# olegroshka/vae-channel-dynamics

Hardware: AMD Instinct MI355X
Metric: images/sec SDXL-VAE train step @256x256 (tracking on) (higher is better)
Workload: dtype f32

## Files before the change

include/vaehip.h:

```cpp
#ifndef VAEHIP_H
#define VAEHIP_H
#include <stdint.h>
#ifdef __cplusplus
extern "C" {
#endif

#define VAE_OK 0
#define VAE_EINVAL (-1)
#define VAE_ELAUNCH (-2)

const char* vae_last_error(void);
int vae_abi_version(void);
int vae_sizeof_args(int32_t which);
int vae_set_option(const char* name, int32_t value);
int vae_get_option(const char* name);

#define VAE_XF_NONE 0
#define VAE_XF_AFFINE 1
#define VAE_XF_AFFINE_SILU 2

#define VAE_PREC_F32 0
#define VAE_PREC_BF16 1

#define VAE_MODE_FWD 0
// ... 59 lines not shown
  const float* scale; const float* shift;
  vae_conv_geom g;
  int32_t M, N;
  int32_t ldy;
  int32_t npix;
  int32_t nsplit;
  int32_t batch; int64_t sYb, sXb, sOb;
  int32_t xf;
  float alpha;
  int32_t prec;
  const void* X16;
  const void* dY16;
  int32_t tapmask;
  int32_t y_step, y_oy, y_ox;
  int32_t x_bf16, y_bf16;
} vae_wgrad_args;
int vae_wgrad(const vae_wgrad_args* a, void* stream);
int vae_wgrad_wino_plan(const vae_wgrad_args* a, int32_t* nsplit);
int vae_wgrad_wino(const vae_wgrad_args* a, void* stream);
int vae_wgrad_wino_reduce(const float* slab, int32_t nsplit, int32_t npos, int32_t Cin, int32_t Cout, float* scratch, float* dW,
                          const float* bias_partial, float* db, void* stream);
int vae_wgrad_wino_positions(const vae_wgrad_args* a);
int vae_wgrad_io16_ok(const vae_wgrad_args* a);
int vae_wgrad_phase_ok(const vae_wgrad_args* a);
int vae_upconv_fold_wgrad(const float* dWeff, const float* dbeff, int32_t Co, int32_t Ci, float* dW, float* db, void* stream);
int vae_wgrad_plan(const vae_wgrad_args* a, int32_t* nsplit, int32_t* xf_fusable);
int vae_igemm_kernel_name(const vae_igemm_args* a, char* buf, int32_t n);
int vae_wgrad_kernel_name(const vae_wgrad_args* a, char* buf, int32_t n);
int vae_reduce_splits(const float* partial, int32_t nsplit, int64_t n, float* out, void* stream);
int vae_reduce_splits2(const float* partial, int32_t nsplit, int64_t n, float* out, const float* partial2, int32_t n2, float* out2,
// ... 78 lines not shown
```

vae-channel-dynamics_amd/csrc/common_host.h:

```cpp
#pragma once
#include <stddef.h>
#include <stdint.h>
#include <hip/hip_runtime_api.h>
#include "../../include/vaehip.h"

void vae_set_error(const char* fmt, ...);

#define VAE_CHECK(cond, ...)                 \
  do {                                       \
    if (!(cond)) {                           \
      vae_set_error(__VA_ARGS__);            \
      return VAE_EINVAL;                     \
    }                                        \
  } while (0)

#define VAE_LAUNCH_CHECK(name)                                                 \
  do {                                                                         \
    hipError_t e_ = hipGetLastError();                                         \
    if (e_ != hipSuccess) {                                                    \
      vae_set_error("%s: launch failed: %s", name, hipGetErrorString(e_));     \
      return VAE_ELAUNCH;                                                      \
    }                                                                          \
  } while (0)

static inline bool aligned16(const void* p) { return (((uintptr_t)p) & 15u) == 0; }

constexpr int SS_HALF = 512;
constexpr size_t BUF_MAX = 0xFFFFFFF0u;

struct vae_options {
  int flat_conv;
  int no_wino;
  int no_wino4;
  int no_thin_mfma;
  int no_wide;
  int no_wgrad_dma;
  int wide_reserved_cus;
};
const vae_options& vae_opt();

#define VAE_RESERVE_LDS(kern, bytes, what)                                                                                  \
  do {                                                                                                                      \
    static unsigned long long done_ = 0;                                                                                    \
    int dev_ = 0;                                                                                                           \
    (void)hipGetDevice(&dev_);                                                                                              \
    if (!((done_ >> (dev_ & 63)) & 1ull)) {                                                                                 \
      if (hipFuncSetAttribute(reinterpret_cast<const void*>(kern), hipFuncAttributeMaxDynamicSharedMemorySize, (int)(bytes)) != hipSuccess) { \
        vae_set_error("%s: cannot reserve %d bytes of LDS", what, (int)(bytes));                                            \
        return VAE_ELAUNCH;                                                                                                 \
      }                                                                                                                     \
// ... 4 lines not shown
```

vae-channel-dynamics_amd/csrc/dispatch.cpp:

```cpp
#include <stdio.h>
#include <algorithm>
#include "launchers.h"

namespace {

constexpr int BK = 32;
const char* const TF[2] = {"false", "true"};

int check_geom(const char* who, const vae_conv_geom& g) {
  VAE_CHECK(g.B > 0 && g.Hs > 0 && g.Ws > 0 && g.Cs > 0 && g.Ho > 0 && g.Wo > 0, "%s: non-positive geometry", who);
  VAE_CHECK(g.taps == 1 || g.taps == 9, "%s: taps must be 1 or 9 (got %d)", who, g.taps);
  VAE_CHECK(g.stride == 1 || g.stride == 2, "%s: stride must be 1 or 2", who);
  VAE_CHECK(g.mode >= 0 && g.mode <= 4, "%s: bad mode", who);
  VAE_CHECK(g.mode != VAE_MODE_UP2X_DGRAD || (g.taps == 9 && g.stride == 1 && g.Hs == 2 * g.Ho && g.Ws == 2 * g.Wo),
            "%s: UP2X_DGRAD needs 3x3 stride 1, source twice the row grid", who);
  VAE_CHECK(g.mode != VAE_MODE_DGRAD_S2 ||
                (g.taps == 9 && g.stride == 2 && g.pad_t == 0 && g.pad_l == 0 && g.Ho % 2 == 0 && g.Wo % 2 == 0 &&
                 ((int64_t)g.B * g.Ho * g.Wo / 4) % 128 == 0),
            "%s: DGRAD_S2 needs 3x3 stride 2 pad 0, even row grid and B*Ho*Wo/4 %% 128 == 0", who);
  VAE_CHECK(g.mode != VAE_MODE_UP2X || (g.taps == 9 && g.stride == 1), "%s: up2x needs 3x3 stride 1", who);
  return 0;
}

bool xf_rows_ok(const vae_conv_geom& g, int M, int K) {
// ... 477 lines not shown
  const char* what = "wgrad";
  switch (s.k) {
    case WgradKernel::DmaBf16: rc = launch_wgrad3_dma_bf16(a, st); what = "wgrad3_dma_bf16"; break;
    case WgradKernel::TileBf16: rc = launch_wgrad3_tile_bf16(a, st); what = "wgrad3_tile_bf16"; break;
    case WgradKernel::Tile: rc = launch_wgrad3_tile(a, st); what = "wgrad3_tile"; break;
    case WgradKernel::ThinBf16: rc = launch_wgrad_thin(a, st); what = "wgrad_thin_bf16"; break;
    case WgradKernel::SmallK: rc = launch_wgrad_smallk(a, st); what = "wgrad_smallk"; break;
    case WgradKernel::Bf16: rc = launch_wgrad_bf16(a, st); what = "wgrad_bf16"; break;
    default: rc = launch_wgrad_f32(a, s.vec, st); break;
  }
  if (rc) return rc;
  VAE_LAUNCH_CHECK(what);
  return VAE_OK;
}

extern "C" int vae_wgrad_wino_plan(const vae_wgrad_args* ap, int32_t* nsplit) {
  VAE_CHECK(ap && nsplit, "wgrad_wino_plan: null argument");
  *nsplit = 0;
  if (vae_opt().flat_conv || vae_opt().no_wino) return VAE_OK;
  const bool up = wgrad3_upwino_eligible(*ap);
  if (!up && !wgrad3_wino_eligible(*ap)) return VAE_OK;
  const int64_t units = up ? wgrad3_upwino_units(ap->g) : wgrad3_wino_units(ap->g);
  const int64_t wgs = (int64_t)(ap->M / 128) * (ap->N / 32);
  *nsplit = (int32_t)std::max<int64_t>(1, std::min<int64_t>(256 / std::max<int64_t>(wgs, 1), units / 8));
  return VAE_OK;
}
extern "C" int vae_wgrad_wino_positions(const vae_wgrad_args* ap) { return (ap && wgrad3_upwino_eligible(*ap)) ? 9 : 16; }
extern "C" int vae_wgrad_wino(const vae_wgrad_args* ap, void* stream) {
  VAE_CHECK(ap != nullptr, "wgrad_wino: null args");
  const vae_wgrad_args& a = *ap;
  if (int e = check_geom("wgrad_wino", a.g)) return e;
  VAE_CHECK(a.dY && a.X && a.partial, "wgrad_wino: null operand");
  VAE_CHECK(a.nsplit > 0 && a.nsplit <= 65535, "wgrad_wino: bad nsplit");
  VAE_CHECK((int64_t)a.g.B * a.g.Ho * a.g.Wo == a.npix && a.N <= a.g.Cs && a.ldy >= a.M, "wgrad_wino: inconsistent sizes");
  const bool up = wgrad3_upwino_eligible(a);
  if (!up) {
    VAE_CHECK(wgrad3_wino_eligible(a), "wgrad_wino: the layer is not served by the Winograd kernel (vae_wgrad_wino_plan)");
    VAE_CHECK(a.xf == VAE_XF_NONE || (a.scale && a.shift), "wgrad_wino: xf needs scale/shift");
  }
  if (int rc = (up ? launch_wgrad3_upwino : launch_wgrad3_wino)(a, (hipStream_t)stream)) return rc;
  VAE_LAUNCH_CHECK(up ? "wgrad3_upwino" : "wgrad3_wino");
  return VAE_OK;
}
```

vae-channel-dynamics_amd/csrc/error.cpp:

```cpp
#include <stdarg.h>
#include <stdio.h>
#include <stdlib.h>
#include <string.h>
#include "common_host.h"

static thread_local char g_err[512] = "";

void vae_set_error(const char* fmt, ...) {
  va_list ap;
  va_start(ap, fmt);
  vsnprintf(g_err, sizeof(g_err), fmt, ap);
  va_end(ap);
}

static vae_options init_options() {
  vae_options o;
  o.flat_conv = getenv("VAEHIP_FLAT_CONV") ? 1 : 0;
  o.no_wino = getenv("VAEHIP_NO_WINO") ? 1 : 0;
  o.no_wide = getenv("VAEHIP_NO_WIDE") ? 1 : 0;
  o.no_wino4 = getenv("VAEHIP_NO_WINO4") ? 1 : 0;
  o.no_thin_mfma = getenv("VAEHIP_NO_THIN_MFMA") ? 1 : 0;
  o.no_wgrad_dma = getenv("VAEHIP_NO_WGRAD_DMA") ? 1 : 0;
  const char* r = getenv("VAEHIP_WIDE_RESERVED_CUS");
  o.wide_reserved_cus = r ? atoi(r) : 0;
  if (o.wide_reserved_cus < 0 || o.wide_reserved_cus > 128) o.wide_reserved_cus = 0;
  return o;
}
static vae_options g_opt = init_options();
const vae_options& vae_opt() { return g_opt; }

static int* option_slot(const char* name) {
  if (!name) return nullptr;
  if (!strcmp(name, "flat_conv")) return &g_opt.flat_conv;
  if (!strcmp(name, "no_wino")) return &g_opt.no_wino;
  if (!strcmp(name, "no_wide")) return &g_opt.no_wide;
  if (!strcmp(name, "no_wino4")) return &g_opt.no_wino4;
  if (!strcmp(name, "no_thin_mfma")) return &g_opt.no_thin_mfma;
  if (!strcmp(name, "no_wgrad_dma")) return &g_opt.no_wgrad_dma;
  if (!strcmp(name, "wide_reserved_cus")) return &g_opt.wide_reserved_cus;
  return nullptr;
}

extern "C" const char* vae_last_error(void) { return g_err; }
extern "C" int vae_abi_version(void) { return 12; }
extern "C" int vae_sizeof_args(int32_t which) {
  return which == 0 ? (int)sizeof(vae_conv_geom) : which == 1 ? (int)sizeof(vae_igemm_args) : which == 2 ? (int)sizeof(vae_wgrad_args) : -1;
}
extern "C" int vae_set_option(const char* name, int32_t value) {
  int* s = option_slot(name);
  if (!s) {
    vae_set_error("set_option: unknown option '%s' (flat_conv, no_wino, no_wino4, no_wide, no_thin_mfma, no_wgrad_dma, wide_reserved_cus)", name ? name : "(null)");
    return VAE_EINVAL;
  }
  if (s == &g_opt.wide_reserved_cus) {
    if (value < 0 || value > 128) {
      vae_set_error("set_option: wide_reserved_cus must be in 0..128, got %d", (int)value);
      return VAE_EINVAL;
    }
    *s = value;
    return VAE_OK;
  }
  *s = value ? 1 : 0;
  return VAE_OK;
}
extern "C" int vae_get_option(const char* name) {
  int* s = option_slot(name);
// ... 3 lines not shown
```

vae-channel-dynamics_amd/csrc/igemm.hip:

```cpp
#include "common.h"
#include <algorithm>
#include <stdlib.h>

#include "launchers.h"

namespace {

constexpr int BK = 32;
__device__ __forceinline__ int b_lo_of(int m0, int hw) { return m0 / hw; }


template <int BM, int BN, int WM, int WN, bool BKM, bool VEC, int XF>
__global__ __launch_bounds__(64 * WM * WN) void igemm_rows_kernel(vae_igemm_args p) {
  constexpr int NT = 64 * WM * WN;
  constexpr int NL = NT;
  constexpr int RP = NT / 8;
  constexpr int LDA = BK + 4;
  constexpr int LDB = BKM ? (BN + 4) : (BK + 4);
  constexpr int SA = BM * LDA;
  constexpr int SB = BKM ? BK * LDB : BN * LDB;
  constexpr int STAGE = SA + SB;
  constexpr int SS = (XF != VAE_XF_NONE) ? 2 * SS_HALF : 0;
  constexpr int TM = BM / WM, TN = BN / WN, MI = TM / 32, NI = TN / 32;
  constexpr int AR = BM / RP;
// ... 580 lines not shown
  VAE_CHECK(partial && out && nsplit > 0 && n > 0, "reduce_splits: bad args");
  if (int rc = reduce_splits_impl(partial, nsplit, n, out, nullptr, 0, nullptr, (hipStream_t)stream)) return rc;
  VAE_LAUNCH_CHECK("reduce_splits");
  return VAE_OK;
}
extern "C" int vae_reduce_splits2(const float* partial, int32_t nsplit, int64_t n, float* out, const float* partial2, int32_t n2, float* out2,
                                  void* stream) {
  VAE_CHECK(partial && out && partial2 && out2 && nsplit > 0 && n > 0 && n2 > 0, "reduce_splits2: bad args");
  if (int rc = reduce_splits_impl(partial, nsplit, n, out, partial2, n2, out2, (hipStream_t)stream)) return rc;
  VAE_LAUNCH_CHECK("reduce_splits2");
  return VAE_OK;
}
extern "C" int vae_wgrad_wino_reduce(const float* slab, int32_t nsplit, int32_t npos, int32_t Cin, int32_t Cout, float* scratch, float* dW,
                                     const float* bias_partial, float* db, void* stream) {
  VAE_CHECK(slab && dW && nsplit > 0 && Cin > 0 && Cout > 0 && Cin % 32 == 0 && Cout % 32 == 0, "wgrad_wino_reduce: bad args");
  VAE_CHECK(npos == 16 || npos == 9, "wgrad_wino_reduce: npos must be 16 (plain 3x3 layer) or 9 (upsampler convolution)");
  VAE_CHECK((bias_partial == nullptr) == (db == nullptr), "wgrad_wino_reduce: bias_partial and db go together");
  VAE_CHECK(nsplit == 1 || scratch != nullptr, "wgrad_wino_reduce: nsplit > 1 needs the [16*Cin*Cout] scratch buffer");
  hipStream_t st = (hipStream_t)stream;
  if (nsplit > 1) {
    if (int rc = reduce_splits_impl(slab, nsplit, (int64_t)npos * Cin * Cout, scratch, bias_partial, bias_partial ? Cout : 0, db, st)) return rc;
    VAE_LAUNCH_CHECK("reduce_splits");
    if (int rc = (npos == 9 ? launch_upwino_wgrad_reduce : launch_wino_wgrad_reduce)(scratch, 1, Cin, Cout, dW, nullptr, nullptr, st)) return rc;
  } else {
    if (int rc = (npos == 9 ? launch_upwino_wgrad_reduce : launch_wino_wgrad_reduce)(slab, 1, Cin, Cout, dW, bias_partial, db, st)) return rc;
  }
  VAE_LAUNCH_CHECK("wino_wgrad_reduce");
  return VAE_OK;
}
```

vae-channel-dynamics_amd/csrc/launchers.h:

```cpp
#pragma once
#include "common_host.h"

int launch_rows_f32(const vae_igemm_args& a, bool bkm, bool vec, hipStream_t st);
int launch_wgrad_f32(const vae_wgrad_args& a, bool vec, hipStream_t st);
int launch_rows_bf16(const vae_igemm_args& a, bool bkm, hipStream_t st);
int launch_wgrad_bf16(const vae_wgrad_args& a, hipStream_t st);

bool conv3_tile_eligible(const vae_igemm_args& a, bool vec, bool bkm);
int conv3_tile_gstat_chunks(const vae_igemm_args& a);
int launch_conv3_tile(const vae_igemm_args& a, bool bkm, hipStream_t st);
bool conv3_tile_bf16_packed(const vae_igemm_args& a);
int conv3_tile_bf16_gstat_chunks(const vae_igemm_args& a);
int launch_conv3_tile_bf16(const vae_igemm_args& a, bool bkm, hipStream_t st);
bool conv3_wide_bf16_eligible(const vae_igemm_args& a);
int conv3_wide_bf16_gstat_chunks(const vae_igemm_args& a);
int launch_conv3_wide_bf16(const vae_igemm_args& a, hipStream_t st);
bool conv3_wino_eligible(const vae_igemm_args& a);
int conv3_wino_nb();
int conv3_wino_gstat_chunks(const vae_igemm_args& a);
int conv3_wino_gnb_chunks(const vae_igemm_args& a);
int launch_wino_weights(const vae_igemm_args& a, float* U, hipStream_t st);
int launch_conv3_wino(const vae_igemm_args& a, const float* U, hipStream_t st);
bool conv3_wino4_eligible(const vae_igemm_args& a);
int conv3_wino4_gstat_chunks(const vae_igemm_args& a);
// ... 19 lines not shown
bool wgrad_thin_bf16_eligible(const vae_wgrad_args& a, int kind);
int launch_wgrad_thin(const vae_wgrad_args& a, hipStream_t st);

bool wgrad3_tile_eligible(const vae_wgrad_args& a, bool vec);
int64_t wgrad3_tile_units(const vae_conv_geom& g);
int launch_wgrad3_tile(const vae_wgrad_args& a, hipStream_t st);
bool wgrad3_dma_bf16_operands(const vae_wgrad_args& a);
bool wgrad3_tile_bf16_eligible(const vae_wgrad_args& a, bool vec, bool dma);
int64_t wgrad3_tile_bf16_units(const vae_conv_geom& g);
int wgrad3_tile_bf16_columns(const vae_wgrad_args& a);
int launch_wgrad3_tile_bf16(const vae_wgrad_args& a, hipStream_t st);
int launch_wgrad3_dma_bf16(const vae_wgrad_args& a, hipStream_t st);
bool wgrad3_wino_eligible(const vae_wgrad_args& a);
int64_t wgrad3_wino_units(const vae_conv_geom& g);
int launch_wgrad3_wino(const vae_wgrad_args& a, hipStream_t st);
int launch_wino_wgrad_reduce(const float* slab, int nsplit, int N, int M, float* dW, const float* bpart, float* db, hipStream_t st);
bool wgrad3_upwino_eligible(const vae_wgrad_args& a);
int64_t wgrad3_upwino_units(const vae_conv_geom& g);
int launch_wgrad3_upwino(const vae_wgrad_args& a, hipStream_t st);
int launch_upwino_wgrad_reduce(const float* slab, int nsplit, int N, int M, float* dW, const float* bpart, float* db, hipStream_t st);
```

vae-channel-dynamics_amd/src/vaehip/engine.py:

```python
from __future__ import annotations

import contextlib
import weakref
from typing import Callable, Dict, List, Optional

import torch
import torch.nn as nn

from . import ops
from .ops import XF_AFFINE, XF_AFFINE_SILU, XF_NONE, Stats

_TRACK_C = {4, 8, 16, 32, 64, 128, 256, 512, 1024}
MOMENT_METRICS = ("mean_abs_activation_per_channel", "mean_activation", "std_activation")
DEVICE_METRICS = MOMENT_METRICS + ("full_activation_map",)


class _TrackHandle:
    def __init__(self, store: dict, key, point: str, sink):
        self._s, self._k, self._p, self._f = store, key, point, sink

    def remove(self):
        lst = self._s.get(self._k, {}).get(self._p, [])
        if self._f in lst:
            lst.remove(self._f)
# ... 239 lines not shown

    def _take16(self, recording: bool) -> Optional[torch.Tensor]:
        a16, self._last16 = self._last16, None
        return a16 if recording else None

    def _conv_bwd(self, m, x, dy, xf, st, need_dx=True, x16=None, dx_to_gn=False, dx_dtype=None, norm=None):
        kind = getattr(m, "kind", "c1")
        gnb = None
        if norm is not None and need_dx and st is not None and xf in (XF_AFFINE, XF_AFFINE_SILU):
            gnb = ops.GnCtx(x, st, norm.weight, norm.bias, xf == XF_AFFINE_SILU, norm.num_groups)
        if (need_dx and dy.dtype == torch.float32 and getattr(dy, "_b16", None) is None
                and ops.grad_image_ok(kind, x.shape[:3] + (m.weight.shape[1],), m.weight.shape[0], m.weight.shape[1])):
            dy._b16 = ops.pack_bf16(dy, torch.empty(dy.shape, device=dy.device, dtype=torch.bfloat16))
        if x16 is not None and x16.dtype == torch.float32:
            x, xf, st, x16 = x16, XF_NONE, None, None
        ops.conv_wgrad(dy, x, kind, self._g(m.weight), self._g(m.bias), xf=xf, stats=st, x16=x16)
        if need_dx:
            return ops.conv_dgrad(dy, m.weight, kind, (x.shape[1], x.shape[2]), out_bf16=dx_to_gn, out_dtype=dx_dtype, gnb=gnb)
        return None

    def _gn_bwd(self, norm, x, g, st, silu, add, conv_only=None, feeds_conv3=False):
        want32, want16 = True, False
        if ops.act16():
            want32, want16 = False, True
        elif conv_only is not None and ops.grad_image_ok(getattr(conv_only, "kind", "c1"), x.shape[:3] + (conv_only.weight.shape[1],),
                                                      conv_only.weight.shape[0], conv_only.weight.shape[1]):
            want32, want16 = False, True
        elif feeds_conv3 and ops.grad_image_ok("c3", x.shape, x.shape[3], x.shape[3]):
            want16 = True
        return ops.gn_bwd(x, g, st, norm.weight, norm.bias, silu, add, self._g(norm.weight), self._g(norm.bias),
                          norm.num_groups, want32=want32, want16=want16)
# ... 346 lines not shown
```

vae-channel-dynamics_amd/src/vaehip/lib.py:

```python
from __future__ import annotations

import ctypes as C
import os

_HERE = os.path.dirname(os.path.abspath(__file__))
LIB_PATH = os.environ.get("VAEHIP_LIB") or os.path.normpath(os.path.join(_HERE, "..", "..", "csrc", "libvaehip.so"))


class VaeHipError(RuntimeError):
    pass


class ConvGeom(C.Structure):
    _fields_ = [("B", C.c_int32), ("Hs", C.c_int32), ("Ws", C.c_int32), ("Cs", C.c_int32),
                ("Ho", C.c_int32), ("Wo", C.c_int32), ("taps", C.c_int32), ("stride", C.c_int32),
                ("pad_t", C.c_int32), ("pad_l", C.c_int32), ("mode", C.c_int32)]


_fp = C.c_void_p


class IgemmArgs(C.Structure):
    _fields_ = [("A", _fp), ("W", _fp), ("C", _fp), ("bias", _fp), ("res", _fp), ("scale", _fp), ("shift", _fp),
                ("track", _fp), ("g", ConvGeom), ("M", C.c_int32), ("N", C.c_int32), ("K", C.c_int32),
# ... 2 lines not shown
                ("xf", C.c_int32), ("alpha", C.c_float), ("prec", C.c_int32), ("Wh", _fp), ("A16", _fp),
                ("tapmask", C.c_int32), ("a_step", C.c_int32), ("a_oy", C.c_int32), ("a_ox", C.c_int32),
                ("c_step", C.c_int32), ("c_oy", C.c_int32), ("c_ox", C.c_int32),
                ("gstat", _fp), ("gstat_groups", C.c_int32), ("Wu", _fp), ("out_bf16", C.c_int32),
                ("a_bf16", C.c_int32), ("res_bf16", C.c_int32),
                ("gnb_x", _fp), ("gnb_mean", _fp), ("gnb_rstd", _fp), ("gnb_gamma", _fp), ("gnb_beta", _fp), ("gnb_ws", _fp),
                ("gnb_groups", C.c_int32), ("gnb_silu", C.c_int32), ("gnb_x_bf16", C.c_int32)]


class WgradArgs(C.Structure):
    _fields_ = [("dY", _fp), ("X", _fp), ("out", _fp), ("partial", _fp), ("bias_partial", _fp), ("scale", _fp), ("shift", _fp),
                ("g", ConvGeom), ("M", C.c_int32), ("N", C.c_int32), ("ldy", C.c_int32), ("npix", C.c_int32),
                ("nsplit", C.c_int32), ("batch", C.c_int32), ("sYb", C.c_int64), ("sXb", C.c_int64),
                ("sOb", C.c_int64), ("xf", C.c_int32), ("alpha", C.c_float), ("prec", C.c_int32), ("X16", _fp), ("dY16", _fp),
                ("tapmask", C.c_int32), ("y_step", C.c_int32), ("y_oy", C.c_int32), ("y_ox", C.c_int32),
                ("x_bf16", C.c_int32), ("y_bf16", C.c_int32)]


i32, i64, f32, vp = C.c_int32, C.c_int64, C.c_float, C.c_void_p
EXPECTED_ABI = 12

SIGNATURES = {
    "vae_set_option": [C.c_char_p, i32],
    "vae_get_option": [C.c_char_p],
    "vae_igemm_rows": [C.POINTER(IgemmArgs), vp],
    "vae_conv_gstat_chunks": [C.POINTER(IgemmArgs)],
    "vae_conv_gnb_chunks": [C.POINTER(IgemmArgs)],
    "vae_conv_phase_ok": [C.POINTER(IgemmArgs)],
    "vae_conv_io16_ok": [C.POINTER(IgemmArgs)],
    "vae_wgrad_io16_ok": [C.POINTER(WgradArgs)],
    "vae_add_bf16": [vp, vp, i64, vp, vp],
    "vae_unpack_bf16": [vp, i64, vp, vp],
    "vae_wino_ok": [C.POINTER(IgemmArgs)],
    "vae_wino_weight_floats": [C.POINTER(IgemmArgs)],
    "vae_wino_weights": [C.POINTER(IgemmArgs), vp, vp],
# ... 101 lines not shown
```

vae-channel-dynamics_amd/src/vaehip/ops.py:

```python
from __future__ import annotations

import ctypes as C
import os
from typing import NamedTuple, Optional, Tuple

import torch

from .lib import ConvGeom, IgemmArgs, WgradArgs, lib

XF_NONE, XF_AFFINE, XF_AFFINE_SILU = 0, 1, 2
PREC_F32, PREC_BF16 = 0, 1
PRECISION = PREC_F32


FUSED_GN_STATS = True

WEIGHTS16: Optional[Tuple[int, int, int]] = None


def pack_bf16(src: torch.Tensor, dst: torch.Tensor) -> torch.Tensor:
    assert src.is_contiguous() and dst.is_contiguous() and dst.numel() == src.numel() and dst.element_size() == 2
    lib.call("vae_pack_bf16", _p(src), src.numel(), _p(dst), _stream())
    return dst

# ... 631 lines not shown
            else:
                a.partial = _p(partial)
            a.bias_partial = _p(bpart)
            _launch_wgrad(a)
            if ns > 1 and bpart is not None:
                lib.call("vae_reduce_splits2", _p(partial), ns, n, _p(dwe[ph]), _p(bpart), Co, _p(dbe[ph]), _stream())
            elif ns > 1:
                lib.call("vae_reduce_splits", _p(partial), ns, n, _p(dwe[ph]), _stream())
            elif bpart is not None:
                lib.call("vae_reduce_splits", _p(bpart), ns, Co, _p(dbe[ph]), _stream())
    lib.call("vae_upconv_fold_wgrad", _p(dwe), _p(dbe), Co, Ci, _p(gv), _p(bgrad_out), _stream())
    del keep
    return True


def _wgrad_wino(a: WgradArgs, gv: torch.Tensor, bgrad_out: Optional[torch.Tensor], dev) -> bool:
    if not WINOGRAD or PRECISION != PREC_F32:
        return False
    ns = C.c_int32(0)
    lib.call("vae_wgrad_wino_plan", C.byref(a), C.byref(ns))
    ns = ns.value
    if ns <= 0:
        return False
    npos = int(lib.query("vae_wgrad_wino_positions", C.byref(a)))
    slab = torch.empty((ns, npos * a.N * a.M), device=dev, dtype=torch.float32)
    bpart = torch.empty((ns, a.M), device=dev, dtype=torch.float32) if bgrad_out is not None else None
    a.nsplit, a.partial, a.bias_partial = ns, _p(slab), _p(bpart)
    fl = 2.0 * a.M * a.N * a.npix * 9
    if npos == 9:
        _timed("wgrad3_upwino_kernel", fl, fl * 0.25, "vae_wgrad_wino", C.byref(a), _stream())
    else:
        _timed(f"wgrad3_wino_kernel<{a.xf}>", fl, fl * WINO_EXECUTED, "vae_wgrad_wino", C.byref(a), _stream())
    scratch = torch.empty((npos * a.N * a.M,), device=dev, dtype=torch.float32) if ns > 1 else None
    _timed("wgrad_wino_reduce (split sum + output transform)", 0.0, 0.0, "vae_wgrad_wino_reduce", _p(slab), ns, npos, a.N, a.M,
           _p(scratch), _p(gv), _p(bpart), _p(bgrad_out), _stream())
    return True


def conv_wgrad(dy: torch.Tensor, x: torch.Tensor, kind: str, wgrad_out: torch.Tensor,
               bgrad_out: Optional[torch.Tensor], *, xf: int = XF_NONE, stats: Optional[Stats] = None,
               x16: Optional[torch.Tensor] = None):
    dy16 = _grad16(dy)
    dy32 = dy if dy.dtype == torch.float32 else None
    _chk_act(dy, "conv_wgrad.dy")
    _chk_act(x, "conv_wgrad.x")
    if x16 is not None:
        assert x16.shape == x.shape and x16.dtype == torch.bfloat16 and x16.is_contiguous()
        xf = XF_NONE
    gv = ohwi(wgrad_out)
    Co, kh, kw, Ci = gv.shape
    taps = kh * kw
    B, H, W, Cs = x.shape
    g = _fwd_geom(kind, B, H, W, Cs)
    assert dy.shape == (B, g.Ho, g.Wo, Co), (dy.shape, (B, g.Ho, g.Wo, Co))
    if (kind == "c3up" and PRECISION == PREC_F32 and WINOGRAD and xf == XF_NONE and x16 is None and dy32 is not None
            and x.dtype == torch.float32):
# ... 13 lines not shown
    a.dY, a.X = _p(dy32 if dy32 is not None else dy16), _p(x)
    a.dY16 = _p(dy16) if use16 else None
    a.g = g
    a.M, a.N, a.ldy, a.npix, a.nsplit = Co, Ci, Co, npix, 1
    a.batch, a.sYb, a.sXb, a.sOb = 1, 0, 0, 0
    a.xf, a.alpha, a.prec = xf, 1.0, PRECISION
    if x16 is not None:
        a.X16 = _p(x16)
    elif xb and xf == XF_NONE:
        a.X16 = _p(x)
    elif xb:
        a.x_bf16 = 1
    if xf != XF_NONE:
        assert stats is not None
        a.scale, a.shift = _p(stats.scale), _p(stats.shift)
    if _wgrad_wino(a, gv, bgrad_out, x.device):
        return
    ns, fus = C.c_int32(0), C.c_int32(0)
    lib.call("vae_wgrad_plan", C.byref(a), C.byref(ns), C.byref(fus))
    if xf != XF_NONE and not fus.value:
        x = gn_apply(x, stats, xf)
        a.X, a.xf, a.scale, a.shift, a.x_bf16 = _p(x), XF_NONE, None, None, 0
        lib.call("vae_wgrad_plan", C.byref(a), C.byref(ns), C.byref(fus))
    if (a.X16 or a.dY16 or a.x_bf16) and not lib.query("vae_wgrad_io16_ok", C.byref(a)):
        x32 = to_f32(x16) if x16 is not None else to_f32(x)
        return conv_wgrad(dy32 if dy32 is not None else to_f32(dy16), x32, kind, wgrad_out, bgrad_out, xf=xf, stats=stats)
    ns = ns.value
    a.nsplit = ns
    partial = None
    if ns == 1:
        a.out = _p(gv)
# ... 318 lines not shown
```

Measured before the change: 103.6.

## Add Winograd F(4x4,3x3) weight-gradient kernel for large f32 3x3 convolutions

Adds a new Winograd F(4,3) weight-gradient path with 36 transform positions for plain stride-1 3x3 f32 layers whose output is at least 64x64. It is used when the engine requests wino4 and no fused GroupNorm transform is involved. A warp-specialised kernel transforms input and output-gradient tiles in LDS and accumulates them with MFMA into split slabs. A second kernel sums the splits and applies the inverse transform to produce dW and db. The goal is fewer multiplies than the existing F(2,3) Winograd path or the direct wgrad on high-resolution layers, at the cost of larger slab and scratch buffers, more transform work, and possible f32 precision loss from the F(4,3) transform constants.

After: 107.2 (median of 6 runs). +3.4%, better.

```diff
diff --git a/include/vaehip.h b/include/vaehip.h
--- a/include/vaehip.h
+++ b/include/vaehip.h
@@ -97,6 +97,7 @@
   int32_t tapmask;
   int32_t y_step, y_oy, y_ox;
   int32_t x_bf16, y_bf16;
+  int32_t wino4;
 } vae_wgrad_args;
 int vae_wgrad(const vae_wgrad_args* a, void* stream);
 int vae_wgrad_wino_plan(const vae_wgrad_args* a, int32_t* nsplit);
diff --git a/vae-channel-dynamics_amd/csrc/common_host.h b/vae-channel-dynamics_amd/csrc/common_host.h
--- a/vae-channel-dynamics_amd/csrc/common_host.h
+++ b/vae-channel-dynamics_amd/csrc/common_host.h
@@ -34,6 +34,7 @@
   int no_wino4;
   int no_thin_mfma;
   int no_wide;
+  int no_wgrad_wino4;
   int no_wgrad_dma;
   int wide_reserved_cus;
 };
diff --git a/vae-channel-dynamics_amd/csrc/dispatch.cpp b/vae-channel-dynamics_amd/csrc/dispatch.cpp
--- a/vae-channel-dynamics_amd/csrc/dispatch.cpp
+++ b/vae-channel-dynamics_amd/csrc/dispatch.cpp
@@ -515,10 +515,18 @@
   return VAE_OK;
 }
 
+static bool wgrad_use_wino4(const vae_wgrad_args& a) {
+  return a.wino4 != 0 && (int64_t)a.g.Ho * a.g.Wo >= 64 * 64 && !vae_opt().flat_conv && !vae_opt().no_wino && !vae_opt().no_wgrad_wino4 && !wgrad3_upwino_eligible(a) &&
+         wgrad3_wino4_eligible(a);
+}
 extern "C" int vae_wgrad_wino_plan(const vae_wgrad_args* ap, int32_t* nsplit) {
   VAE_CHECK(ap && nsplit, "wgrad_wino_plan: null argument");
   *nsplit = 0;
   if (vae_opt().flat_conv || vae_opt().no_wino) return VAE_OK;
+  if (wgrad_use_wino4(*ap)) {
+    *nsplit = wgrad3_wino4_nsplit(*ap);
+    return VAE_OK;
+  }
   const bool up = wgrad3_upwino_eligible(*ap);
   if (!up && !wgrad3_wino_eligible(*ap)) return VAE_OK;
   const int64_t units = up ? wgrad3_upwino_units(ap->g) : wgrad3_wino_units(ap->g);
@@ -526,7 +534,9 @@
   *nsplit = (int32_t)std::max<int64_t>(1, std::min<int64_t>(256 / std::max<int64_t>(wgs, 1), units / 8));
   return VAE_OK;
 }
-extern "C" int vae_wgrad_wino_positions(const vae_wgrad_args* ap) { return (ap && wgrad3_upwino_eligible(*ap)) ? 9 : 16; }
+extern "C" int vae_wgrad_wino_positions(const vae_wgrad_args* ap) {
+  return (ap && wgrad_use_wino4(*ap)) ? 36 : (ap && wgrad3_upwino_eligible(*ap)) ? 9 : 16;
+}
 extern "C" int vae_wgrad_wino(const vae_wgrad_args* ap, void* stream) {
   VAE_CHECK(ap != nullptr, "wgrad_wino: null args");
   const vae_wgrad_args& a = *ap;
@@ -534,6 +544,11 @@
   VAE_CHECK(a.dY && a.X && a.partial, "wgrad_wino: null operand");
   VAE_CHECK(a.nsplit > 0 && a.nsplit <= 65535, "wgrad_wino: bad nsplit");
   VAE_CHECK((int64_t)a.g.B * a.g.Ho * a.g.Wo == a.npix && a.N <= a.g.Cs && a.ldy >= a.M, "wgrad_wino: inconsistent sizes");
+  if (wgrad_use_wino4(a)) {
+    if (int rc = launch_wgrad3_wino4(a, (hipStream_t)stream)) return rc;
+    VAE_LAUNCH_CHECK("wgrad3_wino4");
+    return VAE_OK;
+  }
   const bool up = wgrad3_upwino_eligible(a);
   if (!up) {
     VAE_CHECK(wgrad3_wino_eligible(a), "wgrad_wino: the layer is not served by the Winograd kernel (vae_wgrad_wino_plan)");
diff --git a/vae-channel-dynamics_amd/csrc/error.cpp b/vae-channel-dynamics_amd/csrc/error.cpp
--- a/vae-channel-dynamics_amd/csrc/error.cpp
+++ b/vae-channel-dynamics_amd/csrc/error.cpp
@@ -21,6 +21,7 @@
   o.no_wino4 = getenv("VAEHIP_NO_WINO4") ? 1 : 0;
   o.no_thin_mfma = getenv("VAEHIP_NO_THIN_MFMA") ? 1 : 0;
   o.no_wgrad_dma = getenv("VAEHIP_NO_WGRAD_DMA") ? 1 : 0;
+  o.no_wgrad_wino4 = getenv("VAEHIP_NO_WGRAD_WINO4") ? 1 : 0;
   const char* r = getenv("VAEHIP_WIDE_RESERVED_CUS");
   o.wide_reserved_cus = r ? atoi(r) : 0;
   if (o.wide_reserved_cus < 0 || o.wide_reserved_cus > 128) o.wide_reserved_cus = 0;
@@ -37,19 +38,20 @@
   if (!strcmp(name, "no_wino4")) return &g_opt.no_wino4;
   if (!strcmp(name, "no_thin_mfma")) return &g_opt.no_thin_mfma;
   if (!strcmp(name, "no_wgrad_dma")) return &g_opt.no_wgrad_dma;
+  if (!strcmp(name, "no_wgrad_wino4")) return &g_opt.no_wgrad_wino4;
   if (!strcmp(name, "wide_reserved_cus")) return &g_opt.wide_reserved_cus;
   return nullptr;
 }
 
 extern "C" const char* vae_last_error(void) { return g_err; }
-extern "C" int vae_abi_version(void) { return 12; }
+extern "C" int vae_abi_version(void) { return 13; }
 extern "C" int vae_sizeof_args(int32_t which) {
   return which == 0 ? (int)sizeof(vae_conv_geom) : which == 1 ? (int)sizeof(vae_igemm_args) : which == 2 ? (int)sizeof(vae_wgrad_args) : -1;
 }
 extern "C" int vae_set_option(const char* name, int32_t value) {
   int* s = option_slot(name);
   if (!s) {
-    vae_set_error("set_option: unknown option '%s' (flat_conv, no_wino, no_wino4, no_wide, no_thin_mfma, no_wgrad_dma, wide_reserved_cus)", name ? name : "(null)");
+    vae_set_error("set_option: unknown option '%s' (flat_conv, no_wino, no_wino4, no_wide, no_thin_mfma, no_wgrad_dma, no_wgrad_wino4, wide_reserved_cus)", name ? name : "(null)");
     return VAE_EINVAL;
   }
   if (s == &g_opt.wide_reserved_cus) {
diff --git a/vae-channel-dynamics_amd/csrc/igemm.hip b/vae-channel-dynamics_amd/csrc/igemm.hip
--- a/vae-channel-dynamics_amd/csrc/igemm.hip
+++ b/vae-channel-dynamics_amd/csrc/igemm.hip
@@ -618,10 +618,21 @@
 extern "C" int vae_wgrad_wino_reduce(const float* slab, int32_t nsplit, int32_t npos, int32_t Cin, int32_t Cout, float* scratch, float* dW,
                                      const float* bias_partial, float* db, void* stream) {
   VAE_CHECK(slab && dW && nsplit > 0 && Cin > 0 && Cout > 0 && Cin % 32 == 0 && Cout % 32 == 0, "wgrad_wino_reduce: bad args");
-  VAE_CHECK(npos == 16 || npos == 9, "wgrad_wino_reduce: npos must be 16 (plain 3x3 layer) or 9 (upsampler convolution)");
+  VAE_CHECK(npos == 16 || npos == 9 || npos == 36, "wgrad_wino_reduce: npos must be 16 or 36 (plain 3x3 layer) or 9 (upsampler convolution)");
   VAE_CHECK((bias_partial == nullptr) == (db == nullptr), "wgrad_wino_reduce: bias_partial and db go together");
-  VAE_CHECK(nsplit == 1 || scratch != nullptr, "wgrad_wino_reduce: nsplit > 1 needs the [16*Cin*Cout] scratch buffer");
+  VAE_CHECK(nsplit == 1 || scratch != nullptr, "wgrad_wino_reduce: nsplit > 1 needs the [npos*Cin*Cout] scratch buffer");
   hipStream_t st = (hipStream_t)stream;
+  if (npos == 36) {
+    const float* S = slab;
+    if (nsplit > 1) {
+      if (int rc = reduce_splits_impl(slab, nsplit, (int64_t)npos * Cin * Cout, scratch, bias_partial, bias_partial ? Cout : 0, db, st)) return rc;
+      VAE_LAUNCH_CHECK("reduce_splits");
+      S = scratch;
+    }
+    if (int rc = launch_wino4_wgrad_reduce(S, Cin, Cout, dW, nsplit > 1 ? nullptr : bias_partial, nsplit > 1 ? nullptr : db, st)) return rc;
+    VAE_LAUNCH_CHECK("wino4_wgrad_reduce");
+    return VAE_OK;
+  }
   if (nsplit > 1) {
     if (int rc = reduce_splits_impl(slab, nsplit, (int64_t)npos * Cin * Cout, scratch, bias_partial, bias_partial ? Cout : 0, db, st)) return rc;
     VAE_LAUNCH_CHECK("reduce_splits");
diff --git a/vae-channel-dynamics_amd/csrc/launchers.h b/vae-channel-dynamics_amd/csrc/launchers.h
--- a/vae-channel-dynamics_amd/csrc/launchers.h
+++ b/vae-channel-dynamics_amd/csrc/launchers.h
@@ -57,6 +57,11 @@
 bool wgrad3_wino_eligible(const vae_wgrad_args& a);
 int64_t wgrad3_wino_units(const vae_conv_geom& g);
 int launch_wgrad3_wino(const vae_wgrad_args& a, hipStream_t st);
+bool wgrad3_wino4_eligible(const vae_wgrad_args& a);
+int64_t wgrad3_wino4_units(const vae_conv_geom& g);
+int wgrad3_wino4_nsplit(const vae_wgrad_args& a);
+int launch_wgrad3_wino4(const vae_wgrad_args& a, hipStream_t st);
+int launch_wino4_wgrad_reduce(const float* S, int N, int M, float* dW, const float* bpart, float* db, hipStream_t st);
 int launch_wino_wgrad_reduce(const float* slab, int nsplit, int N, int M, float* dW, const float* bpart, float* db, hipStream_t st);
 bool wgrad3_upwino_eligible(const vae_wgrad_args& a);
 int64_t wgrad3_upwino_units(const vae_conv_geom& g);
diff --git a/vae-channel-dynamics_amd/csrc/wgrad3_wino4.hip b/vae-channel-dynamics_amd/csrc/wgrad3_wino4.hip
--- /dev/null
+++ b/vae-channel-dynamics_amd/csrc/wgrad3_wino4.hip
@@ -0,0 +1,405 @@
+#include "common.h"
+#include <algorithm>
+#include <type_traits>
+
+namespace {
+
+constexpr int QCI = 32, QCO = 64, QNT = 768, QPOS = 36;
+constexpr int QTL = 4;
+constexpr int QHW = 18, QHH = 6;
+constexpr int QHP = QHW * QHH;
+constexpr int QXP = 40;
+constexpr int QSX = QHP * QXP;
+constexpr int QSV = QPOS * QTL * QCI;
+constexpr int QSD = QPOS * QTL * QCO;
+constexpr int QSVD = QSV + QSD;
+constexpr int Q_LDS = (2 * QSX + 2 * QSVD) * 4;
+static_assert(Q_LDS <= 160 * 1024, "LDS");
+
+__device__ __forceinline__ void a6(const float y[4], float z[6]) {
+  const float e = y[0] + y[2], o = y[1] + y[3];
+  const float e2 = fmaf(4.f, y[2], y[0]), o2 = fmaf(8.f, y[3], y[1] + y[1]);
+  z[0] = y[0];
+  z[1] = e + o;
+  z[2] = e - o;
+  z[3] = e2 + o2;
+  z[4] = e2 - o2;
+  z[5] = y[3];
+}
+__device__ __forceinline__ void bt6q(const float r[6], float v[6]) {
+  v[0] = fmaf(4.f, r[0], fmaf(-5.f, r[2], r[4]));
+  const float a = fmaf(-4.f, r[2], r[4]), b = fmaf(-4.f, r[1], r[3]);
+  v[1] = a + b;
+  v[2] = a - b;
+  const float c = r[4] - r[2], e = r[3] - r[1];
+  v[3] = fmaf(2.f, e, c);
+  v[4] = fmaf(-2.f, e, c);
+  v[5] = fmaf(4.f, r[1], fmaf(-5.f, r[3], r[5]));
+}
+
+__global__ __launch_bounds__(QNT, 3) void wgrad3_wino4_kernel(vae_wgrad_args p, int strips, int64_t nunits) {
+  __shared__ __attribute__((aligned(16))) float smem[Q_LDS / 4];
+  float* const sX = smem;
+  float* const sVD = smem + 2 * QSX;
+
+  const int tid = threadIdx.x, lane = tid & 63, wave = __builtin_amdgcn_readfirstlane(tid >> 6);
+  const int lr = lane & 31, lh = lane >> 5;
+  const vae_conv_geom g = p.g;
+  const int tilesN = p.N / QCI, ntile = tilesN * (p.M / QCO);
+  int tile, split;
+  {
+    const int L = blockIdx.x, ns = p.nsplit;
+    if (ns % 8 == 0) {
+      const int j = L >> 3;
+      tile = j % ntile;
+      split = (j / ntile) * 8 + (L & 7);
+    } else if ((ns == 2 || ns == 4) && ntile % (8 / ns) == 0) {
+      split = (L & 7) % ns;
+      tile = (L >> 3) * (8 / ns) + (L & 7) / ns;
+    } else {
+      tile = L % ntile;
+      split = L / ntile;
+    }
+  }
+  const int tm = tile / tilesN, tn = tile % tilesN;
+  const int m0 = tm * QCO, n0 = tn * QCI;
+  const int64_t per = (nunits + p.nsplit - 1) / p.nsplit;
+  const int64_t ubeg = (int64_t)split * per, uend = min(nunits, ubeg + per);
+  const int nu = (int)max((int64_t)0, uend - ubeg);
+  const int upi = (g.Ho / 4) * strips;
+  const bool do_bias = (p.bias_partial != nullptr) && tn == 0;
+
+  struct Unit {
+    int b, ty, x0;
+  };
+  auto unit = [&](int k) __attribute__((always_inline)) {
+    Unit u;
+    if (k >= nu) {
+      u.b = -1; u.ty = 0; u.x0 = 0;
+      return u;
+    }
+    const int i = (int)ubeg + k;
+    const int b = i / upi, r = i - b * upi;
+    u.b = b;
+    u.ty = r / strips;
+    u.x0 = (r - u.ty * strips) * 16;
+    return u;
+  };
+
+  const auto rsX = VAE_BUF_RSRC(p.X, (size_t)g.B * g.Hs * g.Ws * g.Cs * 4u);
+  const auto rsY = VAE_BUF_RSRC(p.dY, (size_t)g.B * g.Ho * g.Wo * p.ldy * 4u);
+
+  f32x16 acc[3][2];
+#pragma unroll
+  for (int pi = 0; pi < 3; ++pi)
+#pragma unroll
+    for (int nb = 0; nb < 2; ++nb)
+#pragma unroll
+      for (int e = 0; e < 16; ++e) acc[pi][nb][e] = 0.f;
+
+  auto mfma_group = [&](const float* c, int pi) __attribute__((always_inline)) {
+    const int pos = 3 * wave + pi;
+    const float* V = c + pos * (QTL * QCI) + lh * QCI + lr;
+    const float* D = c + QSV + pos * (QTL * QCO) + lh * QCO + lr;
+    float a[2], bq[2][2];
+#pragma unroll
+    for (int e = 0; e < 2; ++e) {
+      a[e] = V[2 * e * QCI];
+      bq[0][e] = D[2 * e * QCO];
+      bq[1][e] = D[2 * e * QCO + 32];
+    }
+#pragma unroll
+    for (int nb = 0; nb < 2; ++nb)
+#pragma unroll
+      for (int e = 0; e < 2; ++e) acc[pi][nb] = __builtin_amdgcn_mfma_f32_32x32x2f32(a[e], bq[nb][e], acc[pi][nb], 0, 0, 0);
+  };
+
+  const int xt = tid - 4 * 64;
+  const int xq = xt & 7;
+  int sp[2];
+#pragma unroll
+  for (int j = 0; j < 2; ++j) sp[j] = (xt + 512 * j) >> 3;
+  struct RawX {
+    f32x4 v[2];
+    bool in[2];
+    int b;
+  };
+  auto load_x = [&](int k, RawX& r) __attribute__((always_inline)) {
+    const Unit u = unit(k);
+    r.b = u.b;
+#pragma unroll
+    for (int j = 0; j < 2; ++j) {
+      const int hy = u.ty * 4 - 1 + sp[j] / QHW, hx = u.x0 - 1 + sp[j] % QHW;
+      const bool in = u.b >= 0 && sp[j] < QHP && (unsigned)hy < (unsigned)g.Hs && (unsigned)hx < (unsigned)g.Ws;
+      r.in[j] = in;
+      const unsigned off = (unsigned)((((unsigned)u.b * (unsigned)g.Hs + (unsigned)hy) * (unsigned)g.Ws + (unsigned)hx) * (unsigned)g.Cs +
+                                      (unsigned)(n0 + 4 * xq)) * 4u;
+      r.v[j] = VAE_BUF_LOAD4(rsX, oob_unless(in, off));
+    }
+  };
+  auto store_x = [&](float* dst, const RawX& r) __attribute__((always_inline)) {
+#pragma unroll
+    for (int j = 0; j < 2; ++j)
+      if (sp[j] < QHP) *reinterpret_cast<f32x4*>(&dst[sp[j] * QXP + 4 * xq]) = r.v[j];
+  };
+  const int xw = wave - 4, tp = xw & 1;
+  const int xtile = 2 * tp + lh;
+  const int xsrc = 4 * xtile * QXP + lr;
+  const int vdst = xtile * QCI + lr;
+  auto x_cols = [&](const float* h, auto rg_c, auto c0_c, float (&tr)[2][6]) {
+    constexpr int RG = decltype(rg_c)::value, C0 = decltype(c0_c)::value;
+#pragma unroll
+    for (int j = C0; j < C0 + 3; ++j) {
+      float d[6];
+#pragma unroll
+      for (int i = 0; i < 6; ++i) {
+        const bool need = RG <= 1 ? (i >= 1 && i <= 4) : (RG == 2 ? (i % 2 == 0) : (i % 2 == 1));
+        d[i] = need ? h[xsrc + (i * QHW + j) * QXP] : 0.f;
+      }
+      if (RG == 0) {
+        const float a = fmaf(-4.f, d[2], d[4]), bb = fmaf(-4.f, d[1], d[3]);
+        tr[0][j] = a + bb;
+        tr[1][j] = a - bb;
+      } else if (RG == 1) {
+        const float c = d[4] - d[2], e = d[3] - d[1];
+        tr[0][j] = fmaf(2.f, e, c);
+        tr[1][j] = fmaf(-2.f, e, c);
+      } else if (RG == 2) {
+        tr[0][j] = fmaf(4.f, d[0], fmaf(-5.f, d[2], d[4]));
+      } else {
+        tr[0][j] = fmaf(4.f, d[1], fmaf(-5.f, d[3], d[5]));
+      }
+    }
+  };
+  auto x_rows = [&](float* dst, auto rg_c, const float (&tr)[2][6]) {
+    constexpr int RG = decltype(rg_c)::value;
+    constexpr int NR = RG <= 1 ? 2 : 1;
+#pragma unroll
+    for (int q = 0; q < NR; ++q) {
+      const int I = RG == 0 ? 1 + q : (RG == 1 ? 3 + q : (RG == 2 ? 0 : 5));
+      float v[6];
+      bt6q(tr[q], v);
+#pragma unroll
+      for (int j = 0; j < 6; ++j) dst[(I * 6 + j) * (QTL * QCI) + vdst] = v[j];
+    }
+  };
+
+  const unsigned ythr = (unsigned)(m0 + lane) * 4u;
+  float bsum = 0.f;
+  auto load_y = [&](int k, float (&y)[16]) __attribute__((always_inline)) {
+    const Unit u = unit(k);
+    const bool ok = u.b >= 0;
+    const unsigned vo = ok ? ythr : BUF_OOB;
+    const unsigned base = ok ? (unsigned)((((unsigned)u.b * (unsigned)g.Ho + (unsigned)(4 * u.ty)) * (unsigned)g.Wo + (unsigned)(u.x0 + 4 * wave)) *
+                                          (unsigned)p.ldy) * 4u : 0u;
+    const unsigned rstep = (unsigned)g.Wo * (unsigned)p.ldy * 4u, cstep = (unsigned)p.ldy * 4u;
+#pragma unroll
+    for (int q = 0; q < 16; ++q)
+      y[q] = __builtin_bit_cast(float, __builtin_amdgcn_raw_buffer_load_b32(rsY, vo, ok ? base + (q >> 2) * rstep + (q & 3) * cstep : 0u, 0));
+  };
+  const int ddst = wave * QCO + lane;
+  auto y_rows = [&](float* c, const float (&t)[6][4], auto i0_c) {
+    constexpr int I0 = decltype(i0_c)::value;
+#pragma unroll
+    for (int i = I0; i < I0 + 3; ++i) {
+      float z[6];
+      a6(t[i], z);
+#pragma unroll
+      for (int j = 0; j < 6; ++j) c[QSV + (i * 6 + j) * (QTL * QCO) + ddst] = z[j];
+    }
+  };
+
+  auto run_x = [&](auto rg_c) __attribute__((always_inline)) {
+    RawX rx;
+    load_x(0, rx);
+    store_x(sX, rx);
+    load_x(1, rx);
+    store_x(sX + QSX, rx);
+    load_x(2, rx);
+    __syncthreads();
+    {
+      float tr[2][6];
+      x_cols(sX, rg_c, std::integral_constant<int, 0>{}, tr);
+      x_cols(sX, rg_c, std::integral_constant<int, 3>{}, tr);
+      x_rows(sVD, rg_c, tr);
+    }
+    __syncthreads();
+#pragma unroll 1
+    for (int s = 0; s < nu; ++s) {
+      const int par = s & 1;
+      const float* cur = sVD + par * QSVD;
+      float* nxt = sVD + (par ^ 1) * QSVD;
+      const float* h = sX + (par ^ 1) * QSX;
+      float tr[2][6];
+      store_x(sX + par * QSX, rx);
+      __builtin_amdgcn_sched_barrier(0);
+      load_x(s + 3, rx);
+      x_cols(h, rg_c, std::integral_constant<int, 0>{}, tr);
+      __builtin_amdgcn_sched_barrier(0);
+      mfma_group(cur, 0);
+      __builtin_amdgcn_sched_barrier(0);
+      x_cols(h, rg_c, std::integral_constant<int, 3>{}, tr);
+      __builtin_amdgcn_sched_barrier(0);
+      mfma_group(cur, 1);
+      __builtin_amdgcn_sched_barrier(0);
+      x_rows(nxt, rg_c, tr);
+      __builtin_amdgcn_sched_barrier(0);
+      mfma_group(cur, 2);
+      __syncthreads();
+    }
+  };
+  auto run_y = [&]() __attribute__((always_inline)) {
+    float y[16];
+    float t[6][4];
+    auto cols = [&]() __attribute__((always_inline)) {
+#pragma unroll
+      for (int c = 0; c < 4; ++c) {
+        const float yc[4] = {y[c], y[4 + c], y[8 + c], y[12 + c]};
+        float z[6];
+        a6(yc, z);
+#pragma unroll
+        for (int i = 0; i < 6; ++i) t[i][c] = z[i];
+      }
+      if (do_bias) {
+#pragma unroll
+        for (int q = 0; q < 16; ++q) bsum += y[q];
+      }
+    };
+    load_y(0, y);
+    __syncthreads();
+    cols();
+    load_y(1, y);
+    y_rows(sVD, t, std::integral_constant<int, 0>{});
+    y_rows(sVD, t, std::integral_constant<int, 3>{});
+    __syncthreads();
+#pragma unroll 1
+    for (int s = 0; s < nu; ++s) {
+      const int par = s & 1;
+      const float* cur = sVD + par * QSVD;
+      float* nxt = sVD + (par ^ 1) * QSVD;
+      mfma_group(cur, 0);
+      __builtin_amdgcn_sched_barrier(0);
+      if (s + 1 < nu) cols();
+      y_rows(nxt, t, std::integral_constant<int, 0>{});
+      y_rows(nxt, t, std::integral_constant<int, 3>{});
+      __builtin_amdgcn_sched_barrier(0);
+      load_y(s + 2, y);
+      __builtin_amdgcn_sched_barrier(0);
+      mfma_group(cur, 1);
+      __builtin_amdgcn_sched_barrier(0);
+      mfma_group(cur, 2);
+      __syncthreads();
+    }
+  };
+  if (wave < 4) run_y();
+  else if (xw < 2) run_x(std::integral_constant<int, 0>{});
+  else if (xw < 4) run_x(std::integral_constant<int, 1>{});
+  else if (xw < 6) run_x(std::integral_constant<int, 2>{});
+  else run_x(std::integral_constant<int, 3>{});
+
+  const int el = (int)__builtin_amdgcn_mbcnt_hi(~0u, __builtin_amdgcn_mbcnt_lo(~0u, 0u)), elr = el & 31, elh = el >> 5;
+  float* __restrict__ O = p.partial + (int64_t)split * QPOS * p.N * p.M;
+#pragma unroll
+  for (int pi = 0; pi < 3; ++pi) {
+    const int pos = 3 * wave + pi;
+#pragma unroll
+    for (int nb = 0; nb < 2; ++nb)
+#pragma unroll
+      for (int e = 0; e < 16; ++e) {
+        const int ci = n0 + (e & 3) + 8 * (e >> 2) + 4 * elh;
+        O[((int64_t)pos * p.N + ci) * p.M + m0 + nb * 32 + elr] = acc[pi][nb][e];
+      }
+  }
+  if (do_bias) {
+    if (wave < 4) smem[wave * 64 + el] = bsum;
+    __syncthreads();
+    if (wave == 0) p.bias_partial[(int64_t)split * p.M + m0 + el] = ((smem[el] + smem[64 + el]) + smem[128 + el]) + smem[192 + el];
+  }
+}
+
+__device__ __forceinline__ void gt6(const float m[6], float u[3]) {
+  constexpr float c4 = 0.25f, c6 = 1.0f / 6.0f, c12 = 1.0f / 12.0f, c24 = 1.0f / 24.0f;
+  const float s12 = m[1] + m[2], d12 = m[1] - m[2], s34 = m[3] + m[4], d34 = m[3] - m[4];
+  u[0] = (c4 * m[0] - c6 * s12) + c24 * s34;
+  u[1] = c12 * d34 - c6 * d12;
+  u[2] = (c6 * s34 - c6 * s12) + m[5];
+}
+__global__ __launch_bounds__(256) void wino4_wgrad_reduce_kernel(const float* __restrict__ S, int N, int M, float* __restrict__ dW, int tiles,
+                                                                 const float* __restrict__ bpart, float* __restrict__ db) {
+  __shared__ float sT[9][32][33];
+  const int tid = threadIdx.x;
+  if ((int)blockIdx.x >= tiles) {
+    const int m = ((int)blockIdx.x - tiles) * 256 + tid;
+    if (m < M) db[m] = bpart[m];
+    return;
+  }
+  const int tilesM = M / 32;
+  const int c0 = ((int)blockIdx.x / tilesM) * 32, m0 = ((int)blockIdx.x % tilesM) * 32;
+  const int64_t pstride = (int64_t)N * M;
+#pragma unroll 1
+  for (int r = 0; r < 4; ++r) {
+    const int cl = (tid >> 5) + 8 * r, ml = tid & 31;
+    const float* src = S + (int64_t)(c0 + cl) * M + m0 + ml;
+    float h[3][6];
+#pragma unroll
+    for (int j = 0; j < 6; ++j) {
+      float m[6], u[3];
+#pragma unroll
+      for (int i = 0; i < 6; ++i) m[i] = src[(int64_t)(i * 6 + j) * pstride];
+      gt6(m, u);
+#pragma unroll
+      for (int a = 0; a < 3; ++a) h[a][j] = u[a];
+    }
+#pragma unroll
+    for (int a = 0; a < 3; ++a) {
+      float u[3];
+      gt6(h[a], u);
+#pragma unroll
+      for (int bb = 0; bb < 3; ++bb) sT[a * 3 + bb][ml][cl] = u[bb];
+    }
+  }
+  __syncthreads();
+#pragma unroll 1
+  for (int r = 0; r < 4; ++r) {
+    const int ml = (tid >> 5) + 8 * r, cl = tid & 31;
+#pragma unroll
+    for (int t = 0; t < 9; ++t) dW[((int64_t)(m0 + ml) * 9 + t) * N + c0 + cl] = sT[t][ml][cl];
+  }
+}
+
+}
+
+bool wgrad3_wino4_eligible(const vae_wgrad_args& a) {
+  const vae_conv_geom& g = a.g;
+  if (a.prec != VAE_PREC_F32 || a.X16 != nullptr || a.dY16 != nullptr || a.dY == nullptr || a.batch != 1 || a.alpha != 1.0f) return false;
+  if (a.x_bf16 || a.y_bf16 || a.xf != VAE_XF_NONE) return false;
+  if (g.taps != 9 || g.stride != 1 || g.pad_t != 1 || g.pad_l != 1 || g.mode != VAE_MODE_FWD) return false;
+  if (a.tapmask != 0 || a.y_step > 1 || g.Ho != g.Hs || g.Wo != g.Ws) return false;
+  if (g.Ho % 4 != 0 || g.Wo % 16 != 0 || a.N % QCI != 0 || a.M % QCO != 0 || g.Cs % 4 != 0) return false;
+  if (!aligned16(a.X)) return false;
+  if ((size_t)g.B * g.Hs * g.Ws * g.Cs * 4u >= BUF_MAX || (size_t)g.B * g.Ho * g.Wo * a.ldy * 4u >= BUF_MAX) return false;
+  return true;
+}
+
+int64_t wgrad3_wino4_units(const vae_conv_geom& g) { return (int64_t)g.B * (g.Ho / 4) * (g.Wo / 16); }
+
+int wgrad3_wino4_nsplit(const vae_wgrad_args& a) {
+  const int64_t wgs = (int64_t)(a.M / QCO) * (a.N / QCI);
+  return (int)std::max<int64_t>(1, std::min<int64_t>(256 / std::max<int64_t>(wgs, 1), wgrad3_wino4_units(a.g) / 16));
+}
+
+int launch_wgrad3_wino4(const vae_wgrad_args& a, hipStream_t st) {
+  const vae_conv_geom& g = a.g;
+  const int64_t nunits = wgrad3_wino4_units(g);
+  dim3 grid((unsigned)((a.M / QCO) * (a.N / QCI) * a.nsplit), 1, 1);
+  const int strips = g.Wo / 16;
+  hipLaunchKernelGGL(wgrad3_wino4_kernel, grid, dim3(QNT), 0, st, a, strips, nunits);
+  return 0;
+}
+
+int launch_wino4_wgrad_reduce(const float* S, int N, int M, float* dW, const float* bpart, float* db, hipStream_t st) {
+  const int tiles = (N / 32) * (M / 32);
+  const int extra = bpart ? (M + 255) / 256 : 0;
+  hipLaunchKernelGGL(wino4_wgrad_reduce_kernel, dim3((unsigned)(tiles + extra)), dim3(256), 0, st, S, N, M, dW, tiles, bpart, db);
+  return 0;
+}
diff --git a/vae-channel-dynamics_amd/src/vaehip/engine.py b/vae-channel-dynamics_amd/src/vaehip/engine.py
--- a/vae-channel-dynamics_amd/src/vaehip/engine.py
+++ b/vae-channel-dynamics_amd/src/vaehip/engine.py
@@ -277,7 +277,7 @@
             dy._b16 = ops.pack_bf16(dy, torch.empty(dy.shape, device=dy.device, dtype=torch.bfloat16))
         if x16 is not None and x16.dtype == torch.float32:
             x, xf, st, x16 = x16, XF_NONE, None, None
-        ops.conv_wgrad(dy, x, kind, self._g(m.weight), self._g(m.bias), xf=xf, stats=st, x16=x16)
+        ops.conv_wgrad(dy, x, kind, self._g(m.weight), self._g(m.bias), xf=xf, stats=st, x16=x16, wino4=True)
         if need_dx:
             return ops.conv_dgrad(dy, m.weight, kind, (x.shape[1], x.shape[2]), out_bf16=dx_to_gn, out_dtype=dx_dtype, gnb=gnb)
         return None
diff --git a/vae-channel-dynamics_amd/src/vaehip/lib.py b/vae-channel-dynamics_amd/src/vaehip/lib.py
--- a/vae-channel-dynamics_amd/src/vaehip/lib.py
+++ b/vae-channel-dynamics_amd/src/vaehip/lib.py
@@ -40,11 +40,11 @@
                 ("nsplit", C.c_int32), ("batch", C.c_int32), ("sYb", C.c_int64), ("sXb", C.c_int64),
                 ("sOb", C.c_int64), ("xf", C.c_int32), ("alpha", C.c_float), ("prec", C.c_int32), ("X16", _fp), ("dY16", _fp),
                 ("tapmask", C.c_int32), ("y_step", C.c_int32), ("y_oy", C.c_int32), ("y_ox", C.c_int32),
-                ("x_bf16", C.c_int32), ("y_bf16", C.c_int32)]
+                ("x_bf16", C.c_int32), ("y_bf16", C.c_int32), ("wino4", C.c_int32)]
 
 
 i32, i64, f32, vp = C.c_int32, C.c_int64, C.c_float, C.c_void_p
-EXPECTED_ABI = 12
+EXPECTED_ABI = 13
 
 SIGNATURES = {
     "vae_set_option": [C.c_char_p, i32],
diff --git a/vae-channel-dynamics_amd/src/vaehip/ops.py b/vae-channel-dynamics_amd/src/vaehip/ops.py
--- a/vae-channel-dynamics_amd/src/vaehip/ops.py
+++ b/vae-channel-dynamics_amd/src/vaehip/ops.py
@@ -669,9 +669,10 @@
     return True
 
 
-def _wgrad_wino(a: WgradArgs, gv: torch.Tensor, bgrad_out: Optional[torch.Tensor], dev) -> bool:
+def _wgrad_wino(a: WgradArgs, gv: torch.Tensor, bgrad_out: Optional[torch.Tensor], dev, wino4: bool = False) -> bool:
     if not WINOGRAD or PRECISION != PREC_F32:
         return False
+    a.wino4 = 1 if wino4 else 0
     ns = C.c_int32(0)
     lib.call("vae_wgrad_wino_plan", C.byref(a), C.byref(ns))
     ns = ns.value
@@ -684,6 +685,8 @@
     fl = 2.0 * a.M * a.N * a.npix * 9
     if npos == 9:
         _timed("wgrad3_upwino_kernel", fl, fl * 0.25, "vae_wgrad_wino", C.byref(a), _stream())
+    elif npos == 36:
+        _timed(f"wgrad3_wino4_kernel<{a.xf}>", fl, fl * 36.0 / 144.0, "vae_wgrad_wino", C.byref(a), _stream())
     else:
         _timed(f"wgrad3_wino_kernel<{a.xf}>", fl, fl * WINO_EXECUTED, "vae_wgrad_wino", C.byref(a), _stream())
     scratch = torch.empty((npos * a.N * a.M,), device=dev, dtype=torch.float32) if ns > 1 else None
@@ -694,7 +697,7 @@
 
 def conv_wgrad(dy: torch.Tensor, x: torch.Tensor, kind: str, wgrad_out: torch.Tensor,
                bgrad_out: Optional[torch.Tensor], *, xf: int = XF_NONE, stats: Optional[Stats] = None,
-               x16: Optional[torch.Tensor] = None):
+               x16: Optional[torch.Tensor] = None, wino4: bool = False):
     dy16 = _grad16(dy)
     dy32 = dy if dy.dtype == torch.float32 else None
     _chk_act(dy, "conv_wgrad.dy")
@@ -738,7 +741,7 @@
     if xf != XF_NONE:
         assert stats is not None
         a.scale, a.shift = _p(stats.scale), _p(stats.shift)
-    if _wgrad_wino(a, gv, bgrad_out, x.device):
+    if _wgrad_wino(a, gv, bgrad_out, x.device, wino4=wino4 and xf == XF_NONE):
         return
     ns, fus = C.c_int32(0), C.c_int32(0)
     lib.call("vae_wgrad_plan", C.byref(a), C.byref(ns), C.byref(fus))
```
